# jing2li/MGPreconditionedGCR

Hardware: AMD Instinct MI355X
Metric: gcr_iterations_per_sec (higher is better)
Workload: dtype f64; 1 GPU; 3D 7-point Poisson 128^3 per GPU, unpreconditioned GCR restart 5, complex fp64, x0=0, RHS splitmix64 seed 0; rows=2097152, nnz=14581760, complex=True, stored_matrix_bytes=2097292, ell_width=7, tail_nnz=0, partition=1 GPU

## Files before the change

mgpreconditionedgcr_amd/csrc/gcr_stepbuild.hip:

```cpp
#include <climits>
#include <cstdlib>
#include <type_traits>

#include "internal.h"
#include "reduce.h"
#include "gcr_dev.h"
#include "spmv_dev.h"
#include "exchange_dev.h"

namespace mgcr {

constexpr int SB_MAX_TRIPS = 4;
constexpr int SB_MAX_ND = 5;
constexpr int SB_KEEP_TB = 2;

struct StepBuildArgs {
    RowMat m;
    const cplx *x;
    const cplx *aps[SB_MAX_ND];
    int64_t n;
    int nlogical;
    RowMap rm;
    DevState *st;
    int it;
    const double *partsR;
    int nblkR, strideR;
    double *hist;
    int hist_cap;
    const cplx *den;
    cplx *ap_out;
    double *partsA;
    LeanCoef *lc;
    const cplx *ps[SB_MAX_ND];
    cplx *p_out;
    cplx *xvec;
    cplx *xr_out;
    cplx *xr_den_slot;
    int xr_slot;
    double *partsR_out;
    v4i *slots;
    unsigned gen0;
    unsigned *abort_dev;
    int *abort_host;
    int spin_limit;
    int test_stall;
};

__device__ __forceinline__ cplx sb_xr_alpha(const ResSync &sy, DevState *st, LeanCoef *lc, cplx *xr_den_slot, int xr_slot, int lb) {
    const cplx num = make_double2(res_total(sy, 0), res_total(sy, 1)), den = make_double2(res_total(sy, 2), res_total(sy, 3));
    const cplx alpha = to_sgpr(cdiv(num, den));
    if (lb == 0 && threadIdx.x == 0) {
        *xr_den_slot = den;
        st->npend = xr_slot + 1;
    }
    if (lb == 0 && (int)threadIdx.x < LND) lean_pending_update(lc, xr_slot, alpha, (int)threadIdx.x);
    return alpha;
}

template <int MODE, int WT, int NDT, bool XR, bool CLOSE, bool REALC = false>
__global__ void __launch_bounds__(RED_THREADS, 8) step_build_kernel(StepBuildArgs a) {
    __shared__ double lds[(2 * NDT > 4 ? 2 * NDT : 4) * 17];
    __shared__ double lds_pw[2 * SB_MAX_ND * 17], lds_ws[2 * SB_MAX_ND * RES_GRP];
    __shared__ int gave_up;
    __shared__ cplx sbeta[NDT], scp[NDT];
    extern __shared__ __attribute__((aligned(16))) unsigned char sb_smem[];
    if (a.st->stop_at < a.st->base + a.it) return;
    const int lb = logical_workgroup(a.rm, (int)blockIdx.x, (int)gridDim.x);
    if (lb >= a.nlogical) return;
    cplx *arL = reinterpret_cast<cplx *>(sb_smem);
    ResSync sy;
    res_sync_init(sy, a.slots, a.gen0, a.nlogical, lb, a.abort_dev, a.spin_limit, lds_pw, lds_ws, &gave_up);
    if (a.test_stall && lb == a.test_stall - 1) return;
    int64_t i0, end, stride;
    row_range(a.rm, lb, a.nlogical, a.n, &i0, &end, &stride);
    {
        double v[2 * NDT];
#pragma unroll
        for (int j = 0; j < 2 * NDT; j++) v[j] = 0.;
        int trip = 0;
        for (int64_t i = i0; i < end; i += stride, trip++) {
            const PatLds pl{nullptr, nullptr, nullptr};
            cplx sum;
            if constexpr (REALC) sum = sten_row_product_t<WT, false, 1>(a.m, i, [&](int32_t j) -> cplx { return a.x[j]; });
            else sum = fused_row_product<MODE, WT>(a.m, i, 0, pl, [&](int32_t j) -> cplx { return a.x[j]; });
            const cplx yi = a.m.shift ? csub(a.x[i], cmul(a.m.k, sum)) : sum;
            arL[trip * RED_THREADS + (int)threadIdx.x] = yi;
            __builtin_amdgcn_sched_barrier(0);
            cplx b[NDT];
#pragma unroll
            for (int j = 0; j < NDT; j++) b[j] = ld_stream<true>(a.aps[j] + i);
#pragma unroll
            for (int j = 0; j < NDT; j++) {
                cplx t = cconj_mul(yi, b[j]);
                v[2 * j] += t.x;
                v[2 * j + 1] += t.y;
            }
        }
        const double mine = block_sum_owner<2 * NDT>(v, lds);
        if ((int)threadIdx.x < 2 * NDT) {
            const v4i w4 = {__double2loint(mine), __double2hiint(mine), (int)sy.gen, 0};
            __builtin_amdgcn_raw_buffer_store_b128(w4, sy.slots, ((1 * RES_NV + (int)threadIdx.x) * RES_BLK + lb) * 16, 0, RES_SC1);
        }
    }
    constexpr bool PRE = NDT <= 3;
    cplx pre[NDT];
#pragma unroll
    for (int j = 0; j < NDT; j++) pre[j] = make_double2(0., 0.);
    if (PRE && i0 < end) {
#pragma unroll
        for (int j = 0; j < NDT; j++) pre[j] = ld_stream<NTS>((CLOSE ? a.ps[j] : a.aps[j]) + i0);
    }
    const bool ok = res_collect<2 * NDT>(sy, 1);
    if (!ok) {
        res_abort(a.abort_dev, a.abort_host);
        for (int64_t i = i0; i < end; i += stride) a.ap_out[i] = make_double2(__builtin_nan(""), __builtin_nan(""));
        if ((int)threadIdx.x < 4) a.partsA[threadIdx.x * RED_MAX_BLOCKS + lb] = __builtin_nan("");
        return;
    }
    bool ends_here = false;
    if (XR || lb == 0) {
        double rr[1];
        fold_partials<1>(a.partsR, a.nblkR, a.strideR, rr, lds);
        if (lb == 0 && threadIdx.x == 0) {
            close_step(a.st, a.it, rr[0], a.hist, a.hist_cap, CLOSE);
            if (CLOSE) a.st->closed = 1;
        }
        ends_here = !((rr[0] / a.st->bnorm2) > a.st->tol2);
    }
    if ((int)threadIdx.x < NDT) sbeta[threadIdx.x] = cdiv(make_double2(res_total(sy, 2 * threadIdx.x), res_total(sy, 2 * threadIdx.x + 1)), a.den[threadIdx.x]);
    __syncthreads();
    if constexpr (CLOSE) {
        if ((int)threadIdx.x < NDT) scp[threadIdx.x] = lean_close_coef(a.lc, sbeta, NDT, (int)threadIdx.x);
        __syncthreads();
    }
    if (!CLOSE && lb == 0 && (int)threadIdx.x <= NDT) lean_table_row<NDT>(a.lc, sbeta, (int)threadIdx.x);
    cplx beta[NDT];
#pragma unroll
    for (int j = 0; j < NDT; j++) beta[j] = to_sgpr(sbeta[j]);
    double v[4] = {0., 0., 0., 0.};
    int trip = 0;
    if constexpr (CLOSE) {
        cplx cp[NDT], cx[NDT];
#pragma unroll
        for (int j = 0; j < NDT; j++) {
            cp[j] = to_sgpr(scp[j]);
            cx[j] = to_sgpr(a.lc->cx[j]);
        }
        for (int64_t i = i0; i < end; i += stride) {
            cplx pj[NDT];
#pragma unroll
            for (int j = 0; j < NDT; j++) pj[j] = (PRE && i == i0) ? pre[j] : ld_stream<NTS>(a.ps[j] + i);
            const cplx dv = a.x[i];
            cplx xv = a.xvec[i];
#pragma unroll
            for (int j = 0; j < NDT; j++) xv = cadd(xv, cmul(cx[j], pj[j]));
            a.xvec[i] = xv;
            cplx pc = make_double2(0., 0.);
#pragma unroll
            for (int j = 0; j < NDT; j++) pc = csub(pc, cmul(cp[j], pj[j]));
            st_stream<NTS>(a.p_out + i, cadd(dv, pc));
        }
        __builtin_amdgcn_sched_barrier(0);
    }
    auto build_row = [&](int64_t i, int trip) -> cplx {
        cplx aj[NDT];
#pragma unroll
        for (int j = 0; j < NDT; j++) aj[j] = (PRE && !CLOSE && i == i0) ? pre[j] : ld_stream<NTS>(a.aps[j] + i);
        const cplx av = arL[trip * RED_THREADS + (int)threadIdx.x], rv = a.x[i];
        cplx ac = make_double2(0., 0.);
#pragma unroll
        for (int j = 0; j < NDT; j++) ac = csub(ac, cmul(beta[j], aj[j]));
        const cplx an = cadd(av, ac);
        a.ap_out[i] = an;
        if (XR) arL[trip * RED_THREADS + (int)threadIdx.x] = an;
        cplx t = cconj_mul(rv, an);
        v[0] += t.x; v[1] += t.y;
        cplx u = cconj_mul(an, an);
        v[2] += u.x; v[3] += u.y;
        return rv;
    };
    for (int64_t i = i0; i < end; i += stride, trip++) (void)build_row(i, trip);
    const double mine = block_sum_owner<4>(v, lds);
    if (threadIdx.x < 4) a.partsA[threadIdx.x * RED_MAX_BLOCKS + lb] = mine;
    if constexpr (XR) {
        if ((int)threadIdx.x < 4) {
            const v4i w4 = {__double2loint(mine), __double2hiint(mine), (int)sy.gen, 0};
            __builtin_amdgcn_raw_buffer_store_b128(w4, sy.slots, ((2 * RES_NV + (int)threadIdx.x) * RES_BLK + lb) * 16, 0, RES_SC1);
        }
        const cplx xr0 = i0 < end ? a.x[i0] : make_double2(0., 0.);
        if (!res_collect<4>(sy, 2)) {
            res_abort(a.abort_dev, a.abort_host);
            for (int64_t i = i0; i < end; i += stride) a.xr_out[i] = make_double2(__builtin_nan(""), __builtin_nan(""));
            if (threadIdx.x == 0) a.partsR_out[lb] = __builtin_nan("");
            return;
        }
        if (ends_here) return;
        const cplx alpha = sb_xr_alpha(sy, a.st, a.lc, a.xr_den_slot, a.xr_slot, lb);
        double vr[1] = {0.};
        trip = 0;
        for (int64_t i = i0; i < end; i += stride, trip++) {
            const cplx rn = csub(i == i0 ? xr0 : a.x[i], cmul(alpha, arL[trip * RED_THREADS + (int)threadIdx.x]));
            a.xr_out[i] = rn;
            vr[0] += rn.x * rn.x + rn.y * rn.y;
        }
        const double tot = block_sum_owner<1>(vr, lds);
        if (threadIdx.x == 0) a.partsR_out[lb] = tot;
    }
}

template <class T>
__device__ __forceinline__ T *sb_elem(T *p, uint32_t off) {
    using C = std::conditional_t<std::is_const_v<T>, const char, char>;
    return reinterpret_cast<T *>(reinterpret_cast<C *>(p) + off);
}

__device__ __forceinline__ void sb_wave_pair_to_lds(double (&v)[2], double *lds, int k0) {
    double s;
    const int k = wave_multi_sum<2>(v, s);
    if (((int)threadIdx.x & 31) == 0) lds[(k0 + k) * 17 + ((int)threadIdx.x >> 6)] = s;
}
template <int NV>
__device__ __forceinline__ double sb_block_owner_from_lds(double *lds) {
    const int nwave = (blockDim.x + 63) >> 6;
    __syncthreads();
    double t = 0.;
    if (threadIdx.x < NV)
        for (int w = 0; w < nwave; w++) t += lds[threadIdx.x * 17 + w];
    return t;
}

template <int NDT, bool XR, bool CLOSE, bool REALC>
__global__ void __launch_bounds__(RED_THREADS, 8) step_keep_kernel(StepBuildArgs a) {
    __shared__ double lds[(2 * NDT > 4 ? 2 * NDT : 4) * 17];
    __shared__ double lds_pw[2 * SB_MAX_ND * 17], lds_ws[2 * SB_MAX_ND * RES_GRP];
    __shared__ int gave_up;
    __shared__ cplx sbeta[NDT], scp[NDT], scx[NDT];
    extern __shared__ __attribute__((aligned(16))) unsigned char sb_smem[];
    if (a.st->stop_at < a.st->base + a.it) return;
    const int lb = logical_workgroup(a.rm, (int)blockIdx.x, (int)gridDim.x);
    if (lb >= a.nlogical) return;
    cplx *arL = reinterpret_cast<cplx *>(sb_smem);
    const int tid = (int)threadIdx.x;
    ResSync sy;
    res_sync_init(sy, a.slots, a.gen0, a.nlogical, lb, a.abort_dev, a.spin_limit, lds_pw, lds_ws, &gave_up);
    if (a.test_stall && lb == a.test_stall - 1) return;
    int64_t i0, end, stride;
    row_range(a.rm, lb, a.nlogical, a.n, &i0, &end, &stride);
    auto row = [&](int t) -> int64_t { return i0 + (int64_t)t * stride; };
    uint32_t off[SB_MAX_TRIPS];
#pragma unroll
    for (int t = 0; t < SB_MAX_TRIPS; t++) off[t] = (uint32_t)row(t) * (uint32_t)sizeof(cplx);
    auto at = [&](auto *p, int t) { return sb_elem(p, off[t]); };
    cplx rk[SB_MAX_TRIPS];
#pragma unroll
    for (int t = 0; t < SB_MAX_TRIPS; t++) {
        const int64_t i = row(t);
        rk[t] = make_double2(0., 0.);
        if (i < end) {
            const PatLds pl{nullptr, nullptr, nullptr};
            cplx sum;
            const auto xj = [&](int32_t j) -> cplx { return *sb_elem(a.x, (uint32_t)j * (uint32_t)sizeof(cplx)); };
            if constexpr (REALC) sum = sten_row_product_t<7, false, 1>(a.m, i, xj);
            else sum = fused_row_product<3, 7>(a.m, i, 0, pl, xj);
            rk[t] = *at(a.x, t);
            arL[t * RED_THREADS + tid] = a.m.shift ? csub(rk[t], cmul(a.m.k, sum)) : sum;
        }
        __builtin_amdgcn_sched_barrier(0);
    }
    {
#pragma unroll
        for (int j = 0; j < NDT; j++) {
            cplx b[SB_MAX_TRIPS];
#pragma unroll
            for (int t = 0; t < SB_MAX_TRIPS; t++) b[t] = row(t) < end ? ld_stream<true>(at(a.aps[j], t)) : make_double2(0., 0.);
            double v[2] = {0., 0.};
#pragma unroll
            for (int t = 0; t < SB_MAX_TRIPS; t++) {
                if (row(t) < end) {
                    const cplx tt = cconj_mul(arL[t * RED_THREADS + tid], b[t]);
                    v[0] += tt.x;
                    v[1] += tt.y;
                }
            }
            sb_wave_pair_to_lds(v, lds, 2 * j);
            __builtin_amdgcn_sched_barrier(0);
        }
        const double mine = sb_block_owner_from_lds<2 * NDT>(lds);
        if (tid < 2 * NDT) {
            const v4i w4 = {__double2loint(mine), __double2hiint(mine), (int)sy.gen, 0};
            __builtin_amdgcn_raw_buffer_store_b128(w4, sy.slots, ((1 * RES_NV + tid) * RES_BLK + lb) * 16, 0, RES_SC1);
        }
    }
    cplx pre[SB_KEEP_TB];
#pragma unroll
    for (int u = 0; u < SB_KEEP_TB; u++) pre[u] = row(u) < end ? ld_stream<NTS>(at(a.aps[0], u)) : make_double2(0., 0.);
    if (!res_collect<2 * NDT>(sy, 1)) {
        res_abort(a.abort_dev, a.abort_host);
        for (int64_t i = i0; i < end; i += stride) a.ap_out[i] = make_double2(__builtin_nan(""), __builtin_nan(""));
        if (tid < 4) a.partsA[tid * RED_MAX_BLOCKS + lb] = __builtin_nan("");
        return;
    }
    bool ends_here = false;
    if (XR || lb == 0) {
        double rr[1];
        fold_partials<1>(a.partsR, a.nblkR, a.strideR, rr, lds);
        if (lb == 0 && threadIdx.x == 0) {
            close_step(a.st, a.it, rr[0], a.hist, a.hist_cap, CLOSE);
            if (CLOSE) a.st->closed = 1;
        }
        ends_here = __builtin_amdgcn_readfirstlane(!((rr[0] / a.st->bnorm2) > a.st->tol2)) != 0;
    }
    if (tid < NDT) sbeta[tid] = cdiv(make_double2(res_total(sy, 2 * tid), res_total(sy, 2 * tid + 1)), a.den[tid]);
    __syncthreads();
    if constexpr (CLOSE) {
        if (tid < NDT) {
            scp[tid] = lean_close_coef(a.lc, sbeta, NDT, tid);
            scx[tid] = a.lc->cx[tid];
        }
        __syncthreads();
    }
    if (!CLOSE && lb == 0 && tid <= NDT) lean_table_row<NDT>(a.lc, sbeta, tid);
    {
        cplx beta[NDT];
#pragma unroll
        for (int j = 0; j < NDT; j++) beta[j] = to_sgpr(sbeta[j]);
        double v[4] = {0., 0., 0., 0.};
#pragma unroll
        for (int t0 = 0; t0 < SB_MAX_TRIPS; t0 += SB_KEEP_TB) {
            cplx ac[SB_KEEP_TB];
#pragma unroll
            for (int u = 0; u < SB_KEEP_TB; u++) ac[u] = make_double2(0., 0.);
#pragma unroll
            for (int j = 0; j < NDT; j++) {
                cplx aj[SB_KEEP_TB];
#pragma unroll
                for (int u = 0; u < SB_KEEP_TB; u++)
                    aj[u] = (t0 == 0 && j == 0) ? pre[u] : row(t0 + u) < end ? ld_stream<NTS>(at(a.aps[j], t0 + u)) : make_double2(0., 0.);
#pragma unroll
                for (int u = 0; u < SB_KEEP_TB; u++) ac[u] = csub(ac[u], cmul(beta[j], aj[u]));
                __builtin_amdgcn_sched_barrier(0);
            }
#pragma unroll
            for (int u = 0; u < SB_KEEP_TB; u++) {
                const int t = t0 + u;
                const int64_t i = row(t);
                if (i < end) {
                    const cplx an = cadd(arL[t * RED_THREADS + tid], ac[u]);
                    *at(a.ap_out, t) = an;
                    if (XR) arL[t * RED_THREADS + tid] = an;
                    const cplx tt = cconj_mul(rk[t], an);
                    v[0] += tt.x; v[1] += tt.y;
                    const cplx w = cconj_mul(an, an);
                    v[2] += w.x; v[3] += w.y;
                }
            }
        }
        const double mine = block_sum_owner<4>(v, lds);
        if (tid < 4) a.partsA[tid * RED_MAX_BLOCKS + lb] = mine;
        if (XR && tid < 4) {
            const v4i w4 = {__double2loint(mine), __double2hiint(mine), (int)sy.gen, 0};
            __builtin_amdgcn_raw_buffer_store_b128(w4, sy.slots, ((2 * RES_NV + tid) * RES_BLK + lb) * 16, 0, RES_SC1);
        }
    }
    if constexpr (CLOSE) {
        cplx cx[NDT], cp[NDT];
#pragma unroll
        for (int j = 0; j < NDT; j++) {
            cx[j] = to_sgpr(scx[j]);
            cp[j] = to_sgpr(scp[j]);
        }
#pragma unroll
        for (int t0 = 0; t0 < SB_MAX_TRIPS; t0 += SB_KEEP_TB) {
            cplx xv[SB_KEEP_TB], pc[SB_KEEP_TB];
#pragma unroll
            for (int u = 0; u < SB_KEEP_TB; u++) {
                xv[u] = row(t0 + u) < end ? *at(a.xvec, t0 + u) : make_double2(0., 0.);
                pc[u] = make_double2(0., 0.);
            }
#pragma unroll
            for (int j = 0; j < NDT; j++) {
                cplx pj[SB_KEEP_TB];
#pragma unroll
                for (int u = 0; u < SB_KEEP_TB; u++) pj[u] = row(t0 + u) < end ? ld_stream<NTS>(at(a.ps[j], t0 + u)) : make_double2(0., 0.);
#pragma unroll
                for (int u = 0; u < SB_KEEP_TB; u++) {
                    xv[u] = cadd(xv[u], cmul(cx[j], pj[u]));
                    pc[u] = csub(pc[u], cmul(cp[j], pj[u]));
                }
            }
#pragma unroll
            for (int u = 0; u < SB_KEEP_TB; u++) {
                const int64_t i = row(t0 + u);
                if (i < end) {
                    *at(a.xvec, t0 + u) = xv[u];
                    st_stream<NTS>(at(a.p_out, t0 + u), cadd(rk[t0 + u], pc[u]));
                }
            }
            __builtin_amdgcn_sched_barrier(0);
        }
    }
    if constexpr (XR) {
        if (!res_collect<4>(sy, 2)) {
            res_abort(a.abort_dev, a.abort_host);
            for (int64_t i = i0; i < end; i += stride) a.xr_out[i] = make_double2(__builtin_nan(""), __builtin_nan(""));
            if (threadIdx.x == 0) a.partsR_out[lb] = __builtin_nan("");
            return;
        }
        if (ends_here) return;
        const cplx alpha = sb_xr_alpha(sy, a.st, a.lc, a.xr_den_slot, a.xr_slot, lb);
        double vr[1] = {0.};
#pragma unroll
        for (int t = 0; t < SB_MAX_TRIPS; t++) {
            const int64_t i = row(t);
            if (i < end) {
                const cplx rn = csub(rk[t], cmul(alpha, arL[t * RED_THREADS + tid]));
                *at(a.xr_out, t) = rn;
                vr[0] += rn.x * rn.x + rn.y * rn.y;
            }
        }
        const double tot = block_sum_owner<1>(vr, lds);
        if (threadIdx.x == 0) a.partsR_out[lb] = tot;
    }
}

struct StartArgs {
    RowMat m;
    const cplx *b;
    cplx *ap0;
    int64_t n;
    int nlogical;
    RowMap rm;
    DevState *st;
    double *hist;
    LeanCoef *lc;
    cplx *den0;
    cplx *r_out;
    double *partsR_out;
    v4i *slots;
    unsigned gen0;
    unsigned *abort_dev;
    int *abort_host;
    int spin_limit;
    int test_stall;
};

template <bool REALC>
__global__ void __launch_bounds__(RED_THREADS, 8) start_build_kernel(StartArgs a) {
    __shared__ double lds[6 * 17];
    __shared__ double lds_pw[2 * SB_MAX_ND * 17], lds_ws[2 * SB_MAX_ND * RES_GRP];
    __shared__ int gave_up;
    extern __shared__ __attribute__((aligned(16))) unsigned char sb_smem[];
    if (a.st->stop_at < 0) return;
    const int lb = logical_workgroup(a.rm, (int)blockIdx.x, (int)gridDim.x);
    if (lb >= a.nlogical) return;
    cplx *apL = reinterpret_cast<cplx *>(sb_smem);
    ResSync sy;
    res_sync_init(sy, a.slots, a.gen0, a.nlogical, lb, a.abort_dev, a.spin_limit, lds_pw, lds_ws, &gave_up);
    if (a.test_stall && lb == a.test_stall - 1) return;
    int64_t i0, end, stride;
    row_range(a.rm, lb, a.nlogical, a.n, &i0, &end, &stride);
    {
        double v[6] = {0., 0., 0., 0., 0., 0.};
#pragma unroll
        for (int t = 0; t < SB_MAX_TRIPS; t++) {
            const int64_t i = i0 + (int64_t)t * stride;
            if (i < end) {
                const PatLds pl{nullptr, nullptr, nullptr};
                cplx sum;
                if constexpr (REALC) sum = sten_row_product_t<7, false, 1>(a.m, i, [&](int32_t j) -> cplx { return a.b[j]; });
                else sum = fused_row_product<3, 7>(a.m, i, 0, pl, [&](int32_t j) -> cplx { return a.b[j]; });
                const cplx rv = a.b[i];
                const cplx yi = a.m.shift ? csub(rv, cmul(a.m.k, sum)) : sum;
                a.ap0[i] = yi;
                apL[t * RED_THREADS + (int)threadIdx.x] = yi;
                v[4] += rv.x * rv.x + rv.y * rv.y;
                const cplx tt = cconj_mul(rv, yi);
                v[0] += tt.x; v[1] += tt.y;
                const cplx u = cconj_mul(yi, yi);
                v[2] += u.x; v[3] += u.y;
            }
            __builtin_amdgcn_sched_barrier(0);
        }
        const double mine = block_sum_owner<6>(v, lds);
        if ((int)threadIdx.x < 5) {
            const v4i w4 = {__double2loint(mine), __double2hiint(mine), (int)sy.gen, 0};
            __builtin_amdgcn_raw_buffer_store_b128(w4, sy.slots, ((1 * RES_NV + (int)threadIdx.x) * RES_BLK + lb) * 16, 0, RES_SC1);
        }
    }
    const cplx b0 = i0 < end ? a.b[i0] : make_double2(0., 0.);
    if (!res_collect<5>(sy, 1)) {
        res_abort(a.abort_dev, a.abort_host);
        for (int64_t i = i0; i < end; i += stride) a.r_out[i] = make_double2(__builtin_nan(""), __builtin_nan(""));
        if (threadIdx.x == 0) a.partsR_out[lb] = __builtin_nan("");
        return;
    }
    if (lb == 0 && threadIdx.x == 0) {
        const double nb = res_total(sy, 4);
        a.st->bnorm2 = nb;
        a.st->rr = nb;
        a.hist[0] = sqrt(nb) / sqrt(nb);
    }
    const cplx alpha = sb_xr_alpha(sy, a.st, a.lc, a.den0, 0, lb);
    double vr[1] = {0.};
#pragma unroll
    for (int t = 0; t < SB_MAX_TRIPS; t++) {
        const int64_t i = i0 + (int64_t)t * stride;
        if (i < end) {
            const cplx rn = csub(t == 0 ? b0 : a.b[i], cmul(alpha, apL[t * RED_THREADS + (int)threadIdx.x]));
            a.r_out[i] = rn;
            vr[0] += rn.x * rn.x + rn.y * rn.y;
        }
    }
    const double tot = block_sum_owner<1>(vr, lds);
    if (threadIdx.x == 0) a.partsR_out[lb] = tot;
}

static EnvSwitch g_stepbuild{"MGCR_STEPBUILD"}, g_start_build{"MGCR_START_BUILD"};
static EnvSwitch g_sb_keep_all{"MGCR_SB_KEEP_ALL"};
static EnvSwitch g_sb_real{"MGCR_SB_REAL"};
bool stepbuild_is_enabled() { return g_stepbuild.on(); }
bool set_stepbuild_enabled(bool on) { return g_stepbuild.set(on); }
bool set_start_build_enabled(bool on) { return g_start_build.set(on); }
bool set_stepbuild_keep_all_enabled(bool on) { return g_sb_keep_all.set(on); }
static int64_t g_stepbuild_launches = 0;
int64_t stepbuild_launch_count() { return g_stepbuild_launches; }

template <int NDT, bool XR, bool CLOSE> constexpr bool sb_keep_fits() { return NDT <= 2 || (NDT == 3 && !(XR && CLOSE)); }
template <int NDT, bool XR, bool CLOSE, bool R> const void *sb_keep() {
    if constexpr (sb_keep_fits<NDT, XR, CLOSE>()) return (const void *)step_keep_kernel<NDT, XR, CLOSE, R>;
    else return nullptr;
}
static const void *sb_kernel(int nd, bool xr, bool close, bool realc) {
    if (g_sb_keep_all.on() && nd <= 3) {
#define SKR(NDT, R) (close ? (xr ? sb_keep<NDT, true, true, R>() : sb_keep<NDT, false, true, R>()) \
                           : (xr ? sb_keep<NDT, true, false, R>() : sb_keep<NDT, false, false, R>()))
#define SKK(NDT) (realc ? SKR(NDT, true) : SKR(NDT, false))
        const void *keep = nd == 1 ? SKK(1) : nd == 2 ? SKK(2) : SKK(3);
#undef SKK
#undef SKR
        if (keep) return keep;
    }
#define SBR(NDT, R) (close ? (xr ? (const void *)step_build_kernel<3, 7, NDT, true, true, R> : (const void *)step_build_kernel<3, 7, NDT, false, true, R>) \
                           : (xr ? (const void *)step_build_kernel<3, 7, NDT, true, false, R> : (const void *)step_build_kernel<3, 7, NDT, false, false, R>))
#define SBK(NDT) (realc ? SBR(NDT, true) : SBR(NDT, false))
    switch (nd) {
        case 1: return SBK(1);
        case 2: return SBK(2);
        case 3: return SBK(3);
        case 4: return SBK(4);
        default: return SBK(5);
    }
#undef SBK
#undef SBR
}
bool launch_is_coresident(const void *kernel, int threads, size_t dyn_lds, int grid) {
    struct Key { const void *k; size_t lds; int threads; int per_cu; };
    static std::vector<Key> seen;
    int per_cu = -1;
    for (const Key &e : seen)
        if (e.k == kernel && e.lds == dyn_lds && e.threads == threads) per_cu = e.per_cu;
    if (per_cu < 0) {
        if (dyn_lds > 0) (void)hipFuncSetAttribute(kernel, hipFuncAttributeMaxDynamicSharedMemorySize, (int)(dyn_lds > 64 * 1024 ? dyn_lds : 64 * 1024));
        int nb = 0;
        if (hipOccupancyMaxActiveBlocksPerMultiprocessor(&nb, kernel, threads, dyn_lds) != hipSuccess) { (void)hipGetLastError(); nb = 0; }
        per_cu = nb;
        seen.push_back(Key{kernel, dyn_lds, threads, per_cu});
    }
    static const int force = getenv("MGCR_TEST_OCCUPANCY") ? atoi(getenv("MGCR_TEST_OCCUPANCY")) : -1;
    if (force >= 0) per_cu = force;
    return exchange_shared_init() == MGCR_OK && (int64_t)per_cu * exchange_shared().cus >= grid;
}

static size_t sb_lds_bytes(const CsrDev &A, int g) {
    return sizeof(cplx) * RED_THREADS * (size_t)((A.nrow + (int64_t)g * RED_THREADS - 1) / ((int64_t)g * RED_THREADS));
}

bool csr_step_build_eligible(const CsrDev &A, const DistCsr *dist, int lim) {
    if (!g_stepbuild.on() || dist || comm_live_count() > 0 || lim < 1 || lim > SB_MAX_ND) return false;
    if (!csr_fusable(A, nullptr) || !csr_stencil_active(A) || A.sten_rare || sten_slots(A) != 7) return false;
    const int g = red_grid(A.nrow);
    if (g < 64 || g % 8 != 0) return false;
    if ((int64_t)g * RED_THREADS * SB_MAX_TRIPS < A.nrow) return false;
    if (A.reach >= FUSED_TILE_REACH_DEFAULT) return false;
    if (exchange_shared_init() != MGCR_OK) return false;
    if (g > RES_BLK) return false;
    const size_t lds = sb_lds_bytes(A, g);
    const bool realc = g_sb_real.on() && row_mat(A, false, cplx{0., 0.}).realv;
    for (int xr = 0; xr < 2; xr++)
        for (int cl = 0; cl < 2; cl++)
            if (!launch_is_coresident(sb_kernel(lim, xr != 0, cl != 0, realc), RED_THREADS, lds, g)) return false;
    return true;
}

template <class Args>
static int sb_fill_common(Args &a, const CsrDev &A, bool shift, cplx k, DevState *st, const RowMap &rm, unsigned ngen) {
    MGCR_TRY(exchange_shared_init());
    const ExchangeShared &sh = exchange_shared();
    a.m = row_mat(A, shift, k);
    a.n = A.nrow;
    a.nlogical = red_grid(A.nrow);
    a.rm = rm;
    a.st = st;
    a.slots = sh.slots; a.abort_dev = sh.abort_dev; a.abort_host = sh.abort_host;
    a.gen0 = exchange_take_generations(ngen);
    a.test_stall = getenv("MGCR_TEST_STEPBUILD_STALL") ? atoi(getenv("MGCR_TEST_STEPBUILD_STALL")) : 0;
    a.spin_limit = getenv("MGCR_TEST_RESIDENT_SPIN_LIMIT") ? atoi(getenv("MGCR_TEST_RESIDENT_SPIN_LIMIT")) : RES_SPIN_LIMIT;
    return MGCR_OK;
}
static int sb_launch(const void *kernel, void *args, int grid, size_t lds_bytes, const char *who) {
    MGCR_CHECK(launch_is_coresident(kernel, RED_THREADS, lds_bytes, grid), MGCR_ERR_INVALID, "%s: launch would not be co-resident", who);
    void *kargs[1] = {args};
    MGCR_HIP(hipLaunchKernel(kernel, dim3((unsigned)grid), dim3(RED_THREADS), kargs, lds_bytes, ctx().stream));
    MGCR_HIP(hipGetLastError());
    return MGCR_OK;
}

int csr_step_build(const CsrDev &A, const cplx *x, bool shift, cplx k, const cplx *const *aps, int nd, DevState *st, int it, const double *partsR,
                   int nblkR, int strideR, double *hist, int hist_cap, const cplx *den, cplx *ap_out, double *partsA, LeanCoef *lc,
                   const RowMap &rm, cplx *xr_out, cplx *xr_den_slot, int xr_slot, double *partsR_out, const cplx *const *close_ps, cplx *close_p_out,
                   cplx *close_x) {
    MGCR_CHECK(nd >= 1 && nd <= SB_MAX_ND, MGCR_ERR_INVALID, "csr_step_build: 1..5 directions");
    StepBuildArgs a;
    MGCR_TRY(sb_fill_common(a, A, shift, k, st, rm, 3));
    a.x = x;
    for (int j = 0; j < SB_MAX_ND; j++) a.aps[j] = aps[j < nd ? j : 0];
    a.it = it; a.partsR = partsR; a.nblkR = nblkR; a.strideR = strideR; a.hist = hist; a.hist_cap = hist_cap;
    a.den = den; a.ap_out = ap_out; a.partsA = partsA; a.lc = lc;
    for (int j = 0; j < SB_MAX_ND; j++) a.ps[j] = close_ps ? close_ps[j < nd ? j : 0] : nullptr;
    a.p_out = close_p_out; a.xvec = close_x;
    a.xr_out = xr_out; a.xr_den_slot = xr_den_slot; a.xr_slot = xr_slot; a.partsR_out = partsR_out;
    MGCR_TRY(sb_launch(sb_kernel(nd, xr_out != nullptr, close_ps != nullptr, g_sb_real.on() && a.m.realv), &a, a.nlogical, sb_lds_bytes(A, a.nlogical),
                       "csr_step_build"));
    g_stepbuild_launches++;
    return MGCR_OK;
}

static int64_t g_start_build_launches = 0;
int64_t start_build_launch_count() { return g_start_build_launches; }
static const void *start_kernel(bool realc) {
    return realc ? (const void *)start_build_kernel<true> : (const void *)start_build_kernel<false>;
}

bool csr_start_build_eligible(const CsrDev &A, const DistCsr *dist) {
    if (!g_start_build.on() || !csr_step_build_eligible(A, dist, 1)) return false;
    const bool realc = g_sb_real.on() && row_mat(A, false, cplx{0., 0.}).realv;
    return launch_is_coresident(start_kernel(realc), RED_THREADS, sb_lds_bytes(A, red_grid(A.nrow)), red_grid(A.nrow));
}

int csr_start_build(const CsrDev &A, const cplx *b, bool shift, cplx k, cplx *ap0, DevState *st, double *hist, LeanCoef *lc, cplx *den0,
                    cplx *r_out, double *partsR_out, const RowMap &rm) {
    StartArgs a;
    MGCR_TRY(sb_fill_common(a, A, shift, k, st, rm, 1));
    a.b = b;
    a.ap0 = ap0;
    a.hist = hist; a.lc = lc; a.den0 = den0; a.r_out = r_out; a.partsR_out = partsR_out;
    MGCR_TRY(sb_launch(start_kernel(g_sb_real.on() && a.m.realv), &a, a.nlogical, sb_lds_bytes(A, a.nlogical), "csr_start_build"));
    g_start_build_launches++;
    return MGCR_OK;
}

}
```

Measured before the change: 14400 it/s.

## Merge restart-close row update into build loop and reuse Ap0 loads for beta

For the CLOSE step with NDT==4 (or NDT==5 with XR), the x/p restart update is interleaved into the per-row build loop and reuses the residual row already loaded there. With XR, the last row's close work is deferred until after the partial-sum publish so it overlaps the grid reduction wait. In the stepbuild kernel, the dot-product pass now walks directions in reverse so the aps[0] values it loads are kept in registers (three rows when NDT==1) instead of being reloaded after the sync. This saves a separate streaming pass and some reloads, at the cost of more register pressure and more complex control flow.

```diff
diff --git a/mgpreconditionedgcr_amd/csrc/gcr_stepbuild.hip b/mgpreconditionedgcr_amd/csrc/gcr_stepbuild.hip
--- a/mgpreconditionedgcr_amd/csrc/gcr_stepbuild.hip
+++ b/mgpreconditionedgcr_amd/csrc/gcr_stepbuild.hip
@@ -13,6 +13,8 @@
 constexpr int SB_MAX_TRIPS = 4;
 constexpr int SB_MAX_ND = 5;
 constexpr int SB_KEEP_TB = 2;
+template <int NDT> constexpr int sb_keep_rows() { return NDT == 1 ? 3 : 2; }
+template <int NDT, bool XR, bool CLOSE> constexpr bool sb_close_merged() { return CLOSE && (NDT == 4 || (NDT == 5 && XR)); }
 
 struct StepBuildArgs {
     RowMat m;
@@ -139,7 +141,29 @@
     for (int j = 0; j < NDT; j++) beta[j] = to_sgpr(sbeta[j]);
     double v[4] = {0., 0., 0., 0.};
     int trip = 0;
-    if constexpr (CLOSE) {
+    constexpr bool MERGED = sb_close_merged<NDT, XR, CLOSE>();
+    cplx mcp[MERGED ? NDT : 1], mcx[MERGED ? NDT : 1];
+    if constexpr (MERGED) {
+#pragma unroll
+        for (int j = 0; j < NDT; j++) {
+            mcp[j] = to_sgpr(scp[j]);
+            mcx[j] = to_sgpr(a.lc->cx[j]);
+        }
+    }
+    auto close_row = [&](int64_t i, cplx dv) {
+        cplx pj[NDT];
+#pragma unroll
+        for (int j = 0; j < NDT; j++) pj[j] = ld_stream<NTS>(a.ps[j] + i);
+        cplx xv = a.xvec[i];
+#pragma unroll
+        for (int j = 0; j < NDT; j++) xv = cadd(xv, cmul(mcx[MERGED ? j : 0], pj[j]));
+        a.xvec[i] = xv;
+        cplx pc = make_double2(0., 0.);
+#pragma unroll
+        for (int j = 0; j < NDT; j++) pc = csub(pc, cmul(mcp[MERGED ? j : 0], pj[j]));
+        st_stream<NTS>(a.p_out + i, cadd(dv, pc));
+    };
+    if constexpr (CLOSE && !MERGED) {
         cplx cp[NDT], cx[NDT];
 #pragma unroll
         for (int j = 0; j < NDT; j++) {
@@ -162,11 +186,11 @@
         }
         __builtin_amdgcn_sched_barrier(0);
     }
-    auto build_row = [&](int64_t i, int trip) -> cplx {
+    auto build_row = [&](int64_t i, int trip, cplx r_have) -> cplx {
         cplx aj[NDT];
 #pragma unroll
         for (int j = 0; j < NDT; j++) aj[j] = (PRE && !CLOSE && i == i0) ? pre[j] : ld_stream<NTS>(a.aps[j] + i);
-        const cplx av = arL[trip * RED_THREADS + (int)threadIdx.x], rv = a.x[i];
+        const cplx av = arL[trip * RED_THREADS + (int)threadIdx.x], rv = MERGED ? r_have : a.x[i];
         cplx ac = make_double2(0., 0.);
 #pragma unroll
         for (int j = 0; j < NDT; j++) ac = csub(ac, cmul(beta[j], aj[j]));
@@ -179,14 +203,32 @@
         v[2] += u.x; v[3] += u.y;
         return rv;
     };
-    for (int64_t i = i0; i < end; i += stride, trip++) (void)build_row(i, trip);
+    if constexpr (MERGED) {
+        for (int64_t i = i0; i < end; i += stride, trip++) {
+            const cplx rv = a.x[i];
+            if (!XR || i + stride < end) close_row(i, rv);
+            __builtin_amdgcn_sched_barrier(0);
+            (void)build_row(i, trip, rv);
+            __builtin_amdgcn_sched_barrier(0);
+        }
+    } else {
+        for (int64_t i = i0; i < end; i += stride, trip++) (void)build_row(i, trip, make_double2(0., 0.));
+    }
     const double mine = block_sum_owner<4>(v, lds);
     if (threadIdx.x < 4) a.partsA[threadIdx.x * RED_MAX_BLOCKS + lb] = mine;
+    auto close_last = [&]() {
+        if (trip > 0) {
+            const int64_t il = i0 + (int64_t)(trip - 1) * stride;
+            close_row(il, a.x[il]);
+        }
+        __builtin_amdgcn_sched_barrier(0);
+    };
     if constexpr (XR) {
         if ((int)threadIdx.x < 4) {
             const v4i w4 = {__double2loint(mine), __double2hiint(mine), (int)sy.gen, 0};
             __builtin_amdgcn_raw_buffer_store_b128(w4, sy.slots, ((2 * RES_NV + (int)threadIdx.x) * RES_BLK + lb) * 16, 0, RES_SC1);
         }
+        if constexpr (MERGED) close_last();
         const cplx xr0 = i0 < end ? a.x[i0] : make_double2(0., 0.);
         if (!res_collect<4>(sy, 2)) {
             res_abort(a.abort_dev, a.abort_host);
@@ -267,9 +309,12 @@
         }
         __builtin_amdgcn_sched_barrier(0);
     }
+    constexpr int KT = sb_keep_rows<NDT>();
+    cplx pre[KT];
     {
 #pragma unroll
-        for (int j = 0; j < NDT; j++) {
+        for (int jj = 0; jj < NDT; jj++) {
+            const int j = NDT - 1 - jj;
             cplx b[SB_MAX_TRIPS];
 #pragma unroll
             for (int t = 0; t < SB_MAX_TRIPS; t++) b[t] = row(t) < end ? ld_stream<true>(at(a.aps[j], t)) : make_double2(0., 0.);
@@ -282,6 +327,10 @@
                     v[1] += tt.y;
                 }
             }
+            if (j == 0) {
+#pragma unroll
+                for (int u = 0; u < KT; u++) pre[u] = b[u];
+            }
             sb_wave_pair_to_lds(v, lds, 2 * j);
             __builtin_amdgcn_sched_barrier(0);
         }
@@ -291,9 +340,6 @@
             __builtin_amdgcn_raw_buffer_store_b128(w4, sy.slots, ((1 * RES_NV + tid) * RES_BLK + lb) * 16, 0, RES_SC1);
         }
     }
-    cplx pre[SB_KEEP_TB];
-#pragma unroll
-    for (int u = 0; u < SB_KEEP_TB; u++) pre[u] = row(u) < end ? ld_stream<NTS>(at(a.aps[0], u)) : make_double2(0., 0.);
     if (!res_collect<2 * NDT>(sy, 1)) {
         res_abort(a.abort_dev, a.abort_host);
         for (int64_t i = i0; i < end; i += stride) a.ap_out[i] = make_double2(__builtin_nan(""), __builtin_nan(""));
@@ -335,7 +381,9 @@
                 cplx aj[SB_KEEP_TB];
 #pragma unroll
                 for (int u = 0; u < SB_KEEP_TB; u++)
-                    aj[u] = (t0 == 0 && j == 0) ? pre[u] : row(t0 + u) < end ? ld_stream<NTS>(at(a.aps[j], t0 + u)) : make_double2(0., 0.);
+                    aj[u] = (j == 0 && t0 + u < KT) ? pre[t0 + u < KT ? t0 + u : 0]
+                            : row(t0 + u) < end   ? ld_stream<NTS>(at(a.aps[j], t0 + u))
+                                                  : make_double2(0., 0.);
 #pragma unroll
                 for (int u = 0; u < SB_KEEP_TB; u++) ac[u] = csub(ac[u], cmul(beta[j], aj[u]));
                 __builtin_amdgcn_sched_barrier(0);
```

Result: faster. 14770 it/s, median of 6 (+2.5%).
